# AlerianEmperor/Voxel-Cone-Tracing

Hardware: AMD Instinct MI355X
Metric: Mcones/s (+ ms per GI pass), Sponza-class 256^3 @1080p (higher is better)
Workload: dtype f32; 1 GPU; procedural atrium (Sponza-class, 257488 tris, seed 1234), 256^3 RGBA8 brick chain, 1920x1080, 6 diffuse + 1 specular cone/px, trace of a resident (GPU-rasterised) G-buffer; voxel_dim=256, width=1920, height=1080, cones_per_pixel=7, bounces=1, anisotropic_mips=False, parallelism=single GPU, trace_variant=0, footprint_records=False, comm_reserved_cus=0, raster_form=direct

## Files before the change

include/vct.h:

```cpp
#ifndef VCT_H_
#define VCT_H_

#include <stddef.h>
#include <stdint.h>

#ifdef __cplusplus
extern "C" {
#endif

#define VCT_ABI_VERSION 7

typedef enum vct_status {
    VCT_OK = 0,
    VCT_ERR_INVALID = -1,
    VCT_ERR_DEVICE = -2,
    VCT_ERR_NO_DEVICE = -3,
    VCT_ERR_NOMEM = -4
} vct_status;

enum {
    VCT_GB_POSITION = 0,
    VCT_GB_NORMAL = 3,
    VCT_GB_TANGENT = 6,
    VCT_GB_BITANGENT = 9,
// ... 160 lines not shown
#define VCT_COMM_ID_BYTES 128
int vct_slab_partition(int32_t height, int32_t world, int32_t rank, int32_t* tile_row0, int32_t* tile_row1,
                       int32_t* rows_per_rank);
int vct_comm_get_unique_id(void* id128);
int vct_comm_init(vct_ctx* ctx, const void* id128, int32_t rank, int32_t world);
int vct_comm_destroy(vct_ctx* ctx);
int vct_comm_slab(vct_ctx* ctx, int32_t* tile_row0, int32_t* tile_row1);
int vct_frame_step(vct_ctx* ctx);
int vct_comm_sync(vct_ctx* ctx);
int vct_comm_set_timeout_ms(vct_ctx* ctx, int32_t milliseconds);
int vct_comm_info(vct_ctx* ctx, int32_t out[4]);
int vct_comm_last_gather_ms(vct_ctx* ctx, float* ms);
int vct_last_row_steps(vct_ctx* ctx, uint64_t* rows, int32_t nrows);
int vct_slab_partition_weighted(const uint64_t* row_cost, int32_t tile_rows, int32_t world, int32_t* starts);
int vct_comm_set_slab_rows(vct_ctx* ctx, const int32_t* starts);
int vct_comm_set_interleaved(vct_ctx* ctx, int32_t on);
int vct_selftest_interleaved(vct_ctx* ctx, int32_t world, uint64_t* mismatches);
int vct_comm_frame(vct_ctx* ctx, void** rgba16f_dev, size_t* bytes);
int vct_comm_download_frame(vct_ctx* ctx, void* out_rgba16f_host);

int vct_download_steps(vct_ctx* ctx, uint8_t* steps);
int vct_download_cones(vct_ctx* ctx, float* cones);
int vct_last_step_count(vct_ctx* ctx, uint64_t* steps);
int vct_last_trace_stats(vct_ctx* ctx, uint64_t out[16]);
int vct_get_stage_counts(vct_ctx* ctx, uint64_t out[8]);
int vct_last_trace_ms(vct_ctx* ctx, float* ms);
int vct_set_trace_timing(vct_ctx* ctx, int32_t on);
int vct_selftest_const_divide(vct_ctx* ctx, float d, uint64_t* mismatches);
int vct_selftest_texel_buffer(vct_ctx* ctx, uint64_t* mismatches);
int vct_selftest_area_divide(vct_ctx* ctx, uint64_t seed, uint64_t count, uint64_t* mismatches);
int vct_get_stream(vct_ctx* ctx, void** hip_stream);
int vct_get_frame_device(vct_ctx* ctx, void** rgba16f_dev, size_t* bytes);

#ifdef __cplusplus
}
#endif
#endif
```

voxel-cone-tracing_amd/__init__.py:

```python
import ctypes as C
import os

import numpy as np

try:
    import torch
except ImportError:
    pass

_HERE = os.path.dirname(os.path.abspath(__file__))
LIB_PATH = os.environ.get("VCT_AMD_LIB") or os.path.join(_HERE, "libvct_amd.so")

GB_PLANES = 23
GB_LINEAR, GB_TILED = 0, 1
MEM_HOST, MEM_DEVICE = 0, 1
VOX_CONSERVATIVE_AVG, VOX_REFERENCE = 0, 1
ABI_VERSION = 7
SHOW_DIFFUSE, SHOW_INDIRECT_DIFFUSE, SHOW_SPECULAR, SHOW_INDIRECT_SPECULAR, SHOW_AMBIENT_OCCLUSION = 1, 2, 4, 8, 16
SHOW_ALL = 31
AOV_INDIRECT_DIFFUSE, AOV_INDIRECT_SPECULAR, AOV_DIRECT = 1, 2, 4
VOXVIEW_CURRENT, VOXVIEW_RADIANCE, VOXVIEW_ALBEDO, VOXVIEW_NORMAL = 0, 1, 2, 3
QUERY_SORT_CELLS = 1
POINT_QUERY_MAX = 1 << 26
APERTURE_DIFFUSE, APERTURE_SPECULAR = 0, 1
# ... 556 lines not shown
        v = C.c_int32()
        self._ck(_lib.vct_get_frames_in_flight(self._h, None, None, C.byref(v)), "vct_get_frames_in_flight")
        return bool(v.value)

    def select_frame_slot(self, slot):
        self._ck(_lib.vct_select_frame_slot(self._h, slot), "vct_select_frame_slot")

    def steps(self):
        out = np.zeros((self.cfg.height * self.cfg.width, 7), np.uint8)
        self._ck(_lib.vct_download_steps(self._h, _ptr(out)), "vct_download_steps")
        return out

    def cones(self):
        out = np.zeros((self.cfg.height * self.cfg.width, 7, 4), np.float32)
        self._ck(_lib.vct_download_cones(self._h, _ptr(out)), "vct_download_cones")
        return out

    def last_step_count(self):
        v = C.c_uint64()
        self._ck(_lib.vct_last_step_count(self._h, C.byref(v)), "vct_last_step_count")
        return v.value

    def last_trace_stats(self):
        v = (C.c_uint64 * 16)()
        self._ck(_lib.vct_last_trace_stats(self._h, v), "vct_last_trace_stats")
        keys = ("wave_steps", "lane_steps", "coop_zero", "coop_hit", "fallback", "fallback_lanes", "fallback_fits",
                "greedy_blocks", "greedy_le2", "greedy_le3", "greedy_le4", "quads_live", "quads_fit333", "quads_same",
                "quadrants_live", "quadrants_fit444")
        return dict(zip(keys, (int(x) for x in v)))

    def stage_counts(self):
        v = (C.c_uint64 * 8)()
        self._ck(_lib.vct_get_stage_counts(self._h, v), "vct_get_stage_counts")
        return dict(zip(("triangles", "vox_candidates", "march_division", "accumulator_bricks", "touched_bricks",
                         "comm_reserved_cus", "raster_form", "vox_items"), (int(x) for x in v)))

    def set_trace_timing(self, on=True):
        self._ck(_lib.vct_set_trace_timing(self._h, int(bool(on))), "vct_set_trace_timing")

    def last_trace_ms(self):
        v = C.c_float()
        self._ck(_lib.vct_last_trace_ms(self._h, C.byref(v)), "vct_last_trace_ms")
        return v.value

    def selftest_const_divide(self, d):
        v = C.c_uint64()
        self._ck(_lib.vct_selftest_const_divide(self._h, float(d), C.byref(v)), "vct_selftest_const_divide")
        return v.value

    def selftest_area_divide(self, seed, count):
        v = C.c_uint64()
# ... 17 lines not shown
```

voxel-cone-tracing_amd/csrc/vct_api_trace.hip:

```cpp
#include <algorithm>
#include <map>
#include <mutex>

#include "vct_ctx.h"
#include "vct_divisors.h"

namespace {

int build_steps(const vct_config& cfg, float tan_half, std::vector<VctStep>& out) {
    out.clear();
    const int maxl = vct_ilog2(cfg.voxel_dim);
    const float vs = cfg.grid_world_size / (float)cfg.voxel_dim;
    float dist = vs;
    while (dist < cfg.max_distance) {
        if ((int)out.size() >= VCT_MAX_STEPS) return -1;
        VctStep s;
        const float diameter = fmaxf(vs, 2.0f * tan_half * dist);
        const float lod = log2f(diameter / vs);
        s.dist = dist;
        s.occ_den = 1.0f + 0.03f * diameter;
        s.occ_rcp = 1.0f / s.occ_den;
        float lam = lod;
        if (!(lam > 0.0f)) {
            s.two_levels = 0; s.level = 0; s.level2 = 0; s.frac = 0.0f;
// ... 174 lines not shown
    const uint32_t aov_which = pack_rows ? 0u : c->aov_which;
    const bool half = c->diffuse_rate == 2;
    bool half_march = false;
    if (half) {
        if (row0 != 0 || row1 != vct_tiles_y(c) || row_stride > 1 || pack_rows)
            return vct_fail(c, VCT_ERR_INVALID, "trace: diffuse rate 2 traces whole frames only (no slabs, tile-row ranges or interleaved rows)");
        if (variant != 0 || c->cfg.anisotropic_mips || c->vol.want_cells || c->comm || !cur(c).dr_ind)
            return vct_fail(c, VCT_ERR_INVALID, "trace: diffuse rate 2 needs the default trace kernel on a single-GPU context");
        p.comp = component_word(c->show_mask, aov_which);
        p.aov = aov_which ? cur(c).aov.get() : nullptr;
        half_march = ((p.comp >> VCT_COMP_GROUPS_SHIFT) & 1u) != 0u;
        if (half_march) {
            p.dr_ind = cur(c).dr_ind.get(); p.dr_coarse = cur(c).dr_coarse.get(); p.dr_anchor = cur(c).dr_anchor.get();
            p.dr_list = cur(c).dr_list.get(); p.dr_ctr = cur(c).dr_ctr.get();
            p.dr_waves = c->diffuse_rate_waves;
        }
    } else if (c->show_mask != VCT_SHOW_ALL || aov_which) {
        if (variant != 0)
            return vct_fail(c, VCT_ERR_INVALID, "lighting components / per-component outputs need the default trace kernel (config.trace_variant 0)");
        p.comp = component_word(c->show_mask, aov_which);
        p.aov = aov_which ? cur(c).aov.get() : nullptr;
    }
#if defined(VCT_STATS) && VCT_STATS
    HIP_TRY(c, hipMemsetAsync(c->stats.get(), 0, 16 * sizeof(unsigned long long), cur(c).stream.get()));
#endif
    if (compacting) {
        const size_t nt = (size_t)vct_tiles_x(c) * vct_tiles_y(c);
        HIP_TRY(c, c->vt_pix.reserve(nt * 64 + 4));
        p.vt_pix = c->vt_pix.get();
        p.vt_count = c->vt_pix.get() + nt * 64;
        HIP_TRY(c, hipMemsetAsync(p.vt_count, 0, sizeof(uint32_t), cur(c).stream.get()));
    }
    if (c->time_traces) HIP_TRY(c, hipEventRecord(cur(c).ev0.get(), cur(c).stream.get()));
    const hipEvent_t marks[3] = {cur(c).dr_ev[0].get(), cur(c).dr_ev[1].get(), cur(c).dr_ev[2].get()};
    HIP_TRY(c, vct_launch_trace(p, variant, cur(c).stream.get(), &c->last_march_form,
                                half_march && c->time_traces ? marks : nullptr));
    if (c->time_traces) HIP_TRY(c, hipEventRecord(cur(c).ev1.get(), cur(c).stream.get()));
    cur(c).last_trace_timed = c->time_traces;
    cur(c).last_trace_half = half_march;
    cur(c).last_row0 = row0;
    cur(c).last_row1 = row1;
    cur(c).last_row_stride = rstride;
    cur(c).have_trace = true;
    cur(c).last_was_screen_trace = true;
    cur(c).last_trace_compacted = compacting;
    return VCT_OK;
}
// ... 253 lines not shown
        HIP_TRY(c, hipMemcpy(v, c->step_counter.get(), sizeof(v), hipMemcpyDeviceToHost));
        for (int i = 0; i < VCT_STEP_COUNTERS; ++i) sum += v[i];
    }
    *steps = sum;
    return VCT_OK;
}

int vct_last_row_steps(vct_ctx* c, uint64_t* rows, int32_t nrows) {
    if (!c || !rows) return VCT_ERR_INVALID;
    if (!cur(c).have_trace || !cur(c).last_was_screen_trace)
        return vct_fail(c, VCT_ERR_INVALID, "vct_last_row_steps: the last march was not a screen trace");
    if (nrows != vct_tiles_y(c)) return vct_fail(c, VCT_ERR_INVALID, "vct_last_row_steps: nrows must be the frame's tile rows, ceil(height / 8)");
    if (c->diffuse_rate == 2 || cur(c).last_trace_half)
        return vct_fail(c, VCT_ERR_INVALID, "vct_last_row_steps: diffuse rate 2 keeps no per-row histogram (its marches are not per tile row)");
    if (cur(c).last_trace_compacted)
        return vct_fail(c, VCT_ERR_INVALID, "vct_last_row_steps: the last trace was compacted (config.trace_variant 4): no per-row histogram");
    HIP_TRY(c, hipSetDevice(c->device));
    std::vector<uint64_t> v;
    PIPE_TRY(row_steps(c, v));
    memcpy(rows, v.data(), (size_t)nrows * sizeof(uint64_t));
    return VCT_OK;
}

int vct_last_trace_stats(vct_ctx* c, uint64_t out[16]) {
    if (!c || !out) return VCT_ERR_INVALID;
#if defined(VCT_STATS) && VCT_STATS
    if (!cur(c).have_trace) return vct_fail(c, VCT_ERR_INVALID, "no trace has run");
    HIP_TRY(c, hipStreamSynchronize(cur(c).stream.get()));
    HIP_TRY(c, hipMemcpy(out, c->stats.get(), 16 * sizeof(uint64_t), hipMemcpyDeviceToHost));
    return VCT_OK;
#else
    return vct_fail(c, VCT_ERR_INVALID, "vct_last_trace_stats: this library was built without -DVCT_STATS=1 "
                                    "(tools/build_ab.sh stats \"-DVCT_STATS=1\")");
#endif
}

int vct_last_trace_ms(vct_ctx* c, float* ms) {
    if (!c || !ms) return VCT_ERR_INVALID;
    if (!cur(c).have_trace) return vct_fail(c, VCT_ERR_INVALID, "no trace has run");
    if (!cur(c).last_trace_timed)
        return vct_fail(c, VCT_ERR_INVALID, "vct_last_trace_ms: the last trace was issued with timing off (vct_set_trace_timing)");
    HIP_TRY(c, hipEventSynchronize(cur(c).ev1.get()));
    HIP_TRY(c, hipEventElapsedTime(ms, cur(c).ev0.get(), cur(c).ev1.get()));
    return VCT_OK;
}

int vct_selftest_const_divide(vct_ctx* c, float d, uint64_t* mismatches) {
    if (!c || !mismatches) return VCT_ERR_INVALID;
    if (!divisor_ok(d)) return vct_fail(c, VCT_ERR_INVALID, "divisor outside the set the FMA division is proven for");
    HIP_TRY(c, hipSetDevice(c->device));
    unsigned long long v[2] = {0, 0};
    PIPE_TRY(selftest_words(c, v, [&](unsigned long long* w, hipStream_t st) { return vct_launch_divide_selftest(d, w, st); }));
// ... 171 lines not shown
```

voxel-cone-tracing_amd/csrc/vct_capi.hip:

```cpp
#include <map>
#include <mutex>
#include <utility>

#include "vct_ctx.h"

namespace {

std::string g_create_error;

bool is_pow2(int v) { return v > 0 && (v & (v - 1)) == 0; }

__global__ void k_spin_stamp(long long ticks, unsigned long long* out) {
    const long long t0 = (long long)wall_clock64();
    while ((long long)wall_clock64() - t0 < ticks) __builtin_amdgcn_s_sleep(16);
    out[0] = wall_clock64();
}
__global__ void k_stamp(unsigned long long* out) { out[1] = wall_clock64(); }

int streams_overlap(vct_ctx* c, hipStream_t base, hipStream_t cand, bool* overlap) {
    int khz = 0;
    if (hipDeviceGetAttribute(&khz, hipDeviceAttributeWallClockRate, c->device) != hipSuccess || khz <= 0) khz = 100000;
    HIP_TRY(c, hipMemsetAsync(c->stats.get(), 0, 2 * sizeof(unsigned long long), base));
    HIP_TRY(c, hipStreamSynchronize(base));
    hipLaunchKernelGGL(k_spin_stamp, dim3(1), dim3(1), 0, base, (long long)khz * 3 / 10, c->stats.get());
// ... 51 lines not shown
    HIP_TRY(c, slot_create(c, c->slots[0], stream));
    const char* rp = getenv("VCT_RASTER_PATH");
    c->raster_form.mode = !rp ? 0 : (rp[0] == 'b' ? 2 : (rp[0] == 'd' ? 1 : 0));
    for (VctEvent& ev : c->raster_form.ev) HIP_TRY(c, ev.create());
    if (const char* fr = getenv("VCT_FOOTPRINT_RECORDS")) c->vol.want_cells = fr[0] == '1';
    if (const char* tc = getenv("VCT_BIN_TEST_CAPS")) {
        unsigned a = 0, b = 0;
        if (sscanf(tc, "%u,%u", &a, &b) == 2) { c->raster_form.bin_test_caps[0] = a; c->raster_form.bin_test_caps[1] = b; }
    }
    VctChain& vol = c->vol;
    vol.V = cfg->voxel_dim;
    vol.nlev = vct_ilog2(vol.V) + 1;
    vol.chain_texels = vct_chain_texels(vol.V);
    HIP_TRY(c, vol.chain.alloc(vol.chain_texels));
    HIP_TRY(c, hipMemsetAsync(vol.chain.get(), 0, vol.chain_texels * 4, cur(c).stream.get()));
    const size_t npix = (size_t)cfg->width * cfg->height;
    if (cfg->anisotropic_mips) {
        const size_t n = 6 * (vol.chain_texels - vol.nvox());
        HIP_TRY(c, vol.aniso.alloc(n));
        HIP_TRY(c, hipMemsetAsync(vol.aniso.get(), 0, n * 4, cur(c).stream.get()));
    }
    HIP_TRY(c, c->step_counter.alloc(VCT_STEP_COUNTERS));
    HIP_TRY(c, hipMemsetAsync(c->step_counter.get(), 0, VCT_STEP_COUNTERS * sizeof(unsigned long long), cur(c).stream.get()));
    HIP_TRY(c, c->stats.alloc(16));
    HIP_TRY(c, hipMemsetAsync(c->stats.get(), 0, 16 * sizeof(unsigned long long), cur(c).stream.get()));
    HIP_TRY(c, c->steps_dev.alloc(2 * VCT_MAX_STEPS));
    {
        std::vector<uint32_t> lut(1024);
        for (uint32_t i = 0; i < 1024u; ++i) lut[i] = vct_spread3(i) << 2;
        HIP_TRY(c, c->spread_lut.alloc(lut.size()));
        HIP_TRY(c, hipMemcpy(c->spread_lut.get(), lut.data(), lut.size() * sizeof(uint32_t), hipMemcpyHostToDevice));
    }
    if (cfg->debug_outputs) {
        HIP_TRY(c, c->dbg_steps.alloc(npix * 7));
        HIP_TRY(c, c->dbg_cones.alloc(npix * 28));
        HIP_TRY(c, hipMemsetAsync(c->dbg_steps.get(), 0, npix * 7, cur(c).stream.get()));
        HIP_TRY(c, hipMemsetAsync(c->dbg_cones.get(), 0, npix * 28 * sizeof(float), cur(c).stream.get()));
    }
    HIP_TRY(c, hipStreamSynchronize(cur(c).stream.get()));
    static std::mutex lock;
    static std::map<int, unsigned long long> verdict;
    std::lock_guard<std::mutex> g(lock);
    auto it = verdict.find(c->device);
    if (it == verdict.end()) {
        uint64_t bad = 0;
        PIPE_TRY(vct_selftest_texel_buffer(c, &bad));
        it = verdict.emplace(c->device, bad).first;
    }
// ... 283 lines not shown
```

voxel-cone-tracing_amd/csrc/vct_trace.hip:

```cpp
#include <hip/hip_fp16.h>

#include "../../include/vct.h"
#include "vct_internal.h"
#include "vct_texel.h"


namespace {

struct F3 { float x, y, z; };
struct F4 { float x, y, z, w; };

__device__ __forceinline__ F3 f3(float x, float y, float z) { return {x, y, z}; }
__device__ __forceinline__ float dot3(F3 a, F3 b) { return a.x * b.x + a.y * b.y + a.z * b.z; }
__device__ __forceinline__ F3 cross3(F3 a, F3 b) {
    return {a.y * b.z - a.z * b.y, a.z * b.x - a.x * b.z, a.x * b.y - a.y * b.x};
}
__device__ __forceinline__ float div_rn(float a, float b) { return a / b; }
__device__ __forceinline__ float sqrt_rn(float a) { return __builtin_sqrtf(a); }
__device__ __forceinline__ F3 normalize3(F3 a) {
    const float l = sqrt_rn(dot3(a, a));
    return {div_rn(a.x, l), div_rn(a.y, l), div_rn(a.z, l)};
}
__device__ __forceinline__ F3 reflect3(F3 I, F3 N) {
    const float d = 2.0f * dot3(N, I);
// ... 37 lines not shown
__device__ __forceinline__ float unorm8_of(uint32_t t) {
    if (LOOSE) return (float)((t >> SHIFT) & 0xffu) * 0x1.010102p-8f;
    return vct_unorm8_to_float((t >> SHIFT) & 0xffu);
}

#ifndef VCT_STATS
#define VCT_STATS 0
#endif
struct MarchStats {
    uint32_t wave_steps;
    uint32_t lane_steps;
    uint32_t coop_zero;
    uint32_t coop_hit;
    uint32_t fallback;
    uint32_t fallback_lanes;
    uint32_t fallback_fits;
    uint32_t greedy_blocks, greedy_le2, greedy_le3, greedy_le4;
    uint32_t two_blocks;
    uint32_t quads_live;
    uint32_t quads_fit333;
    uint32_t quads_same;
    uint32_t quadrants_live;
    uint32_t quadrants_fit444;
};

template <bool WRAP, bool COOP, bool LOOSE = false, bool CELLS = false, bool PRIO = false>
__device__ __forceinline__ F4 sample_level(const uint32_t* __restrict__ chain, const VctLevelRef lv,
                                           float ux, float uy, float uz, bool act, unsigned long long am,
                                           float4* __restrict__ blk, const LaneBlock& lb, MarchStats& ms,
                                           const char* __restrict__ cells = nullptr) {
    if (PRIO) __builtin_amdgcn_s_setprio(1);
    const int m = lv.m;
    const float fN = lv.fN;
    const float u = fmaf(ux, fN, -0.5f), v = fmaf(uy, fN, -0.5f), w = fmaf(uz, fN, -0.5f);
    const float fu = floorf(u), fv = floorf(v), fw = floorf(w);
    const float a = u - fu, b = v - fv, c = w - fw;
    const int i0 = (int)fu, j0 = (int)fv, k0 = (int)fw;
    const uint32_t* __restrict__ base = chain + lv.off;
    const uint32_t MX = lv.mask_x, MY = MX << 1, MZ = MX << 2;
    const vct_v4i32 tb = level_texel_buffer(base);

    F4 r = {0.0f, 0.0f, 0.0f, 0.0f};
    bool coop = false;
    int ax = 0, ay = 0, az = 0, dx = 0, dy = 0, dz = 0;
    if (COOP) {
        const int src = ((am >> 27) & 1ull) ? 27 : (int)__ffsll((long long)am) - 1;
        ax = __builtin_amdgcn_readlane(i0, src) - 1;
// ... 7 lines not shown
    if (COOP && coop) {
        uint32_t idx;
        if (WRAP) {
            const uint32_t m4 = (uint32_t)m << 2;
            const uint32_t sax = spread_byte(lb.lut, ax, m4) >> 2;
            const uint32_t say = spread_byte(lb.lut, ay, m4) >> 1;
            const uint32_t saz = spread_byte(lb.lut, az, m4);
            idx = (((sax | ~MX) + lb.sbx) & MX) | (((say | ~MY) + lb.sby) & MY) |
                  (((saz | ~MZ) + lb.sbz) & MZ);
        } else {
            const int x = min(max(ax + (lb.lane & 3), 0), m);
            const int y = min(max(ay + ((lb.lane >> 2) & 3), 0), m);
            const int z = min(max(az + (lb.lane >> 4), 0), m);
            idx = vct_morton3((uint32_t)x, (uint32_t)y, (uint32_t)z);
        }
        const float4 d = texel_f32(tb, idx);
        if (PRIO) __builtin_amdgcn_s_setprio(0);
        const bool any_texel = ballot64((__float_as_uint(d.x) | __float_as_uint(d.y) | __float_as_uint(d.z) | __float_as_uint(d.w)) != 0u) != 0ull;
        if (VCT_STATS) { if (any_texel) ++ms.coop_hit; else ++ms.coop_zero; }
        if (any_texel) {
            blk[lb.lane] = d;
            wave_sync();
            const int slot = act ? (dz * 4 + dy) * 4 + dx : 0;
            const float4* q = blk + slot;
            const float a0 = 1.0f - a, b0 = 1.0f - b, c0 = 1.0f - c;
            const float ab00 = a0 * b0, ab10 = a * b0, ab01 = a0 * b, ab11 = a * b;
            {
                const float4 t0 = q[0], t1 = q[1], t2 = q[4], t3 = q[5];
                const float w0 = ab00 * c0, w1 = ab10 * c0, w2 = ab01 * c0, w3 = ab11 * c0;
#define VCT_ACC(ch) r.ch = w0 * t0.ch; r.ch = fmaf(w1, t1.ch, r.ch); r.ch = fmaf(w2, t2.ch, r.ch); r.ch = fmaf(w3, t3.ch, r.ch);
                VCT_ACC(x) VCT_ACC(y) VCT_ACC(z) VCT_ACC(w)
#undef VCT_ACC
            }
            __builtin_amdgcn_sched_barrier(0);
            {
                const float4 t4 = q[16], t5 = q[17], t6 = q[20], t7 = q[21];
                wave_sync();
                const float w4 = ab00 * c, w5 = ab10 * c, w6 = ab01 * c, w7 = ab11 * c;
#define VCT_ACC(ch) r.ch = fmaf(w4, t4.ch, r.ch); r.ch = fmaf(w5, t5.ch, r.ch); r.ch = fmaf(w6, t6.ch, r.ch); r.ch = fmaf(w7, t7.ch, r.ch);
                VCT_ACC(x) VCT_ACC(y) VCT_ACC(z) VCT_ACC(w)
#undef VCT_ACC
            }
        }
    } else {
      if (VCT_STATS) {
          ++ms.fallback; ms.fallback_lanes += (uint32_t)__popcll(am);
          int lo[3] = {act ? i0 : 0x7fffffff, act ? j0 : 0x7fffffff, act ? k0 : 0x7fffffff};
          int hi[3] = {act ? i0 : -0x7fffffff, act ? j0 : -0x7fffffff, act ? k0 : -0x7fffffff};
          for (int off = 32; off > 0; off >>= 1)
              for (int q = 0; q < 3; ++q) { lo[q] = min(lo[q], __shfl_xor(lo[q], off)); hi[q] = max(hi[q], __shfl_xor(hi[q], off)); }
          if (hi[0] - lo[0] <= 2 && hi[1] - lo[1] <= 2 && hi[2] - lo[2] <= 2) ++ms.fallback_fits;
          unsigned long long pending = am;
          int nb = 0;
          while (pending != 0ull && nb < 16) {
              const int src = (int)__ffsll((long long)pending) - 1;
              const int bx = __builtin_amdgcn_readlane(i0, src) - 1, by = __builtin_amdgcn_readlane(j0, src) - 1,
                        bz = __builtin_amdgcn_readlane(k0, src) - 1;
              const bool in = (uint32_t)(i0 - bx) <= 2u && (uint32_t)(j0 - by) <= 2u && (uint32_t)(k0 - bz) <= 2u;
              pending &= ~ballot64(in);
              ++nb;
          }
          int qlo[3] = {act ? i0 : 0x7fffffff, act ? j0 : 0x7fffffff, act ? k0 : 0x7fffffff};
          int qhi[3] = {act ? i0 : -0x7fffffff, act ? j0 : -0x7fffffff, act ? k0 : -0x7fffffff};
          bool qany = act;
          auto widen = [&](int off) {
// ... 85 lines not shown
                t[6] = base[mx0 | my1 | mz1]; t[7] = base[mx1 | my1 | mz1];
            }
            if (PRIO) __builtin_amdgcn_s_setprio(0);
            const float a0 = 1.0f - a, b0 = 1.0f - b, c0 = 1.0f - c;
            const float wg[8] = {(a0 * b0) * c0, (a * b0) * c0, (a0 * b) * c0, (a * b) * c0,
                                 (a0 * b0) * c,  (a * b0) * c,  (a0 * b) * c,  (a * b) * c};
            r.x = wg[0] * unorm8_of<0, LOOSE>(t[0]);
            r.y = wg[0] * unorm8_of<8, LOOSE>(t[0]);
            r.z = wg[0] * unorm8_of<16, LOOSE>(t[0]);
            r.w = wg[0] * unorm8_of<24, LOOSE>(t[0]);
#pragma unroll
            for (int i = 1; i < 8; ++i) {
                r.x = fmaf(wg[i], unorm8_of<0, LOOSE>(t[i]), r.x);
                r.y = fmaf(wg[i], unorm8_of<8, LOOSE>(t[i]), r.y);
                r.z = fmaf(wg[i], unorm8_of<16, LOOSE>(t[i]), r.z);
                r.w = fmaf(wg[i], unorm8_of<24, LOOSE>(t[i]), r.w);
            }
        }
      }
    }
    return r;
}

struct AnisoCone {
    float wx, wy, wz;
    bool nx, ny, nz;
};

template <bool WRAP, bool COOP>
__device__ __forceinline__ F4 sample_aniso(const VctTraceParams& p, const VctLevelRef lv, float ux,
                                           float uy, float uz, bool act, unsigned long long m,
                                           float4* __restrict__ blk, const LaneBlock& lb, const AnisoCone& ac,
                                           MarchStats& ms) {
    auto chain_of = [&](int d) { return p.aniso + (size_t)d * p.aniso_stride - p.level_off[1]; };
    const unsigned long long mx = ballot64(ac.nx) & m, my = ballot64(ac.ny) & m, mz = ballot64(ac.nz) & m;
    F4 tx, ty, tz;
    bool done = false;
    if (COOP && WRAP) {
        const int mm = lv.m;
        const float fN = lv.fN;
        const float u = fmaf(ux, fN, -0.5f), v = fmaf(uy, fN, -0.5f), w = fmaf(uz, fN, -0.5f);
        const float fu = floorf(u), fv = floorf(v), fw = floorf(w);
        const float a = u - fu, b = v - fv, c = w - fw;
        const int i0 = (int)fu, j0 = (int)fv, k0 = (int)fw;
        const int src = ((m >> 27) & 1ull) ? 27 : (int)__ffsll((long long)m) - 1;
        const int ax = __builtin_amdgcn_readlane(i0, src) - 1;
// ... 75 lines not shown
    r.w = ac.wx * tx.w; r.w = fmaf(ac.wy, ty.w, r.w); r.w = fmaf(ac.wz, tz.w, r.w);
    return r;
}

typedef const __attribute__((address_space(4))) VctStep* StepTable;

__device__ __forceinline__ VctStep load_step(StepTable t, int k) {
    VctStep s;
    s.dist = t[k].dist; s.occ_rcp = t[k].occ_rcp; s.occ_den = t[k].occ_den; s.frac = t[k].frac;
    s.level = t[k].level; s.level2 = t[k].level2; s.two_levels = t[k].two_levels; s.omf = t[k].omf;
    s.l1.off = t[k].l1.off; s.l1.mask_x = t[k].l1.mask_x; s.l1.fN = t[k].l1.fN; s.l1.m = t[k].l1.m;
    s.l2.off = t[k].l2.off; s.l2.mask_x = t[k].l2.mask_x; s.l2.fN = t[k].l2.fN; s.l2.m = t[k].l2.m;
    return s;
}

#define VCT_MARCH_STEP(st, act, live)                                                                        \
        const float px = start.x + dir.x * st.dist; \
        const float py = start.y + dir.y * st.dist; \
        const float pz = start.z + dir.z * st.dist; \
        const float ux = fmaf(div_const<FASTDIV>(px, p.half_G_aux, p.half_G_rcp), 0.5f, 0.5f); \
        const float uy = fmaf(div_const<FASTDIV>(py, p.half_G_aux, p.half_G_rcp), 0.5f, 0.5f); \
        const float uz = fmaf(div_const<FASTDIV>(pz, p.half_G_aux, p.half_G_rcp), 0.5f, 0.5f); \
        F4 vc = (ANISO && st.level >= 1) ? sample_aniso<WRAP, COOP>(p, st.l1, ux, uy, uz, act, live, blk, lb, ac, ms) \
                                         : sample_level<WRAP, COOP, FASTDIV == 2, CELLS, PRIO>(p.chain, st.l1, ux, uy, uz, act, live, blk, lb, ms, p.cells_biased); \
        if (st.two_levels) { \
            const F4 t2 = ANISO ? sample_aniso<WRAP, COOP>(p, st.l2, ux, uy, uz, act, live, blk + 64, lb, ac, ms) \
                                : sample_level<WRAP, COOP, FASTDIV == 2, CELLS, PRIO>(p.chain, st.l2, ux, uy, uz, act, live, blk + 64, lb, ms, p.cells_biased); \
            const float g = st.omf;       \
            vc.x = fmaf(st.frac, t2.x, g * vc.x); \
            vc.y = fmaf(st.frac, t2.y, g * vc.y); \
            vc.z = fmaf(st.frac, t2.z, g * vc.z); \
            vc.w = fmaf(st.frac, t2.w, g * vc.w); \
        } \
        if (act) { \
            const float oma = 1.0f - alpha; \
            cr = fmaf(oma, vc.x, cr); \
            cg = fmaf(oma, vc.y, cg); \
            cb = fmaf(oma, vc.z, cb); \
            occ = occ + div_const<FASTDIV>(oma * vc.w, st.occ_den, st.occ_rcp); \
            alpha = fmaf(oma, vc.w, alpha); \
            ++steps; \
        }

template <bool WRAP, int FASTDIV, bool COOP, bool ANISO = false, bool CELLS = false, bool PRIO = false>
__device__ __forceinline__ F4 cone_march(const VctTraceParams& p, bool alive, F3 start, F3 dir,
                                         const VctStep* tab_global, int n,
                                         float4* __restrict__ blk, const LaneBlock& lb,
                                         int& steps_out, MarchStats& ms) {
    const StepTable tab = (StepTable)tab_global;
    float cr = 0.0f, cg = 0.0f, cb = 0.0f, occ = 0.0f;
    int steps = 0;
    AnisoCone ac = {0.0f, 0.0f, 0.0f, false, false, false};
    if (ANISO) {
        ac.wx = dir.x * dir.x; ac.wy = dir.y * dir.y; ac.wz = dir.z * dir.z;
        ac.nx = !(dir.x >= 0.0f); ac.ny = !(dir.y >= 0.0f); ac.nz = !(dir.z >= 0.0f);
    }
    const float wx = start.x + dir.x * p.vs, wy = start.y + dir.y * p.vs, wz = start.z + dir.z * p.vs;
    float alpha = fmaf(wx, 0.0f, fmaf(wy, 0.0f, fmaf(wz, 0.0f, 0.0f)));
    const unsigned long long alive_mask = ballot64(alive);
    if constexpr (!ANISO) {
    auto march_step = [&](const VctStep& st, const bool act, const unsigned long long live) { VCT_MARCH_STEP(st, act, live) };
    VctStep ea = load_step(tab, 0), eb = ea;
    for (int k = 0; k < n;) {
        {
            const bool act = alive && (alpha < p.max_alpha);
            const unsigned long long live = ballot64(alpha < p.max_alpha) & alive_mask;
            if (live == 0ull) break;
            if (VCT_STATS) { ++ms.wave_steps; ms.lane_steps += (uint32_t)__popcll(live); }
            eb = load_step(tab, k + 1 < n ? k + 1 : k);
            march_step(ea, act, live);
            if (++k >= n) break;
// ... 8 lines not shown
            ++k;
        }
    }
    } else {
    VctStep nxt = load_step(tab, 0);
    for (int k = 0; k < n; ++k) {
        const bool act = alive && (alpha < p.max_alpha);
        const unsigned long long live = ballot64(alpha < p.max_alpha) & alive_mask;
        if (live == 0ull) break;
        if (VCT_STATS) { ++ms.wave_steps; ms.lane_steps += (uint32_t)__popcll(live); }
        const VctStep st = nxt;
        nxt = load_step(tab, k + 1 < n ? k + 1 : k);
        VCT_MARCH_STEP(st, act, live)
    }
    }
    if (alive && steps == 0 && alpha != alpha && n > 0 && 0.0f < p.max_alpha) {
        cr = cg = cb = occ = __builtin_nanf("");
        steps = 1;
    }
    steps_out = steps;
    return {cr, cg, cb, occ};
}

__device__ __forceinline__ void flush_stats(const VctTraceParams& p, const MarchStats& ms, int lane) {
    if (VCT_STATS && p.stats && lane == 0) {
        const uint32_t v[16] = {ms.wave_steps, ms.lane_steps, ms.coop_zero, ms.coop_hit, ms.fallback,
                                ms.fallback_lanes, ms.fallback_fits, ms.greedy_blocks, ms.greedy_le2, ms.greedy_le3,
                                ms.greedy_le4, ms.quads_live, ms.quads_fit333, ms.quads_same, ms.quadrants_live,
                                ms.quadrants_fit444};
        for (int i = 0; i < 16; ++i)
            if (v[i]) atomicAdd(p.stats + i, (unsigned long long)v[i]);
    }
}

__constant__ float kConeDirs[18] = {0.0f, 0.0f, 1.0f,
                                    0.0f, 0.866025f, 0.5f,
                                    0.823639f, 0.267617f, 0.5f,
                                    0.509037f, -0.700629f, 0.5f,
                                    -0.509037f, -0.700629f, 0.5f,
                                    -0.823639f, 0.267617f, 0.5f};
__constant__ float kConeWeights[6] = {0.25f, 0.15f, 0.15f, 0.15f, 0.15f, 0.15f};

__device__ __forceinline__ LaneBlock make_lane_block(const VctTraceParams& p, int lane) {
    LaneBlock lb;
    lb.lane = lane;
    lb.lut = (SpreadLut)p.spread_lut; lb.lut_vec = p.spread_lut;
    lb.sbx = vct_spread3((uint32_t)lane & 3u);
    lb.sby = vct_spread3(((uint32_t)lane >> 2) & 3u) << 1;
// ... 201 lines not shown
    __shared__ int lds_done;
    __shared__ int lds_steps;
    const int lane = threadIdx.x & 63;
    const int wave = __builtin_amdgcn_readfirstlane((int)(threadIdx.x >> 6));
    float4* blk = &lds_blk[wave][0][0];
    if (threadIdx.x == 0) { lds_done = 0; lds_steps = 0; }
    __syncthreads();

    const int ntiles = p.ntiles;
    const int ti = xcd_remap((int)blockIdx.x, (int)gridDim.x);
    if (ti >= ntiles) return;
    constexpr bool compact = COMPACT;
    uint32_t cpix = 0u;
    if (compact) {
        if ((uint32_t)ti >= *p.vt_count) {
            if (threadIdx.x == 0) p.tile_steps[p.tile_row0 * p.tiles_x + ti] = 0u;
            return;
        }
        cpix = p.vt_pix[(size_t)ti * 64 + lane];
    }

    const LaneBlock lb = make_lane_block(p, lane);
    MarchStats ms = {};

    int lrow = 0, tile0 = p.tile_row0 * p.tiles_x + ti;
    if (p.row_stride > 1) {
        lrow = ti / p.tiles_x;
        tile0 = (p.tile_row0 + lrow * p.row_stride) * p.tiles_x + (ti - lrow * p.tiles_x);
    }
    const bool cvalid = !compact || cpix != 0xffffffffu;
    const int tile = compact ? (cvalid ? (int)(cpix >> 6) : 0) : tile0;
    const int ty = tile / p.tiles_x, tx = tile - ty * p.tiles_x;
    const int oy = p.pack_rows ? (p.row_stride > 1 ? lrow : ty - p.tile_row0) : ty;
    const int plane_ = compact ? (int)(cpix & 63u) : lane;
    auto fresh_lane = [&]() { int l = plane_; asm volatile("" : "+v"(l)); return l; };
    auto pixel_index = [&]() {
        const int l = fresh_lane();
        return (size_t)(oy * VCT_TILE + (l >> 3)) * p.width + (tx * VCT_TILE + (l & 7));
    };
    auto gbuf_ptr = [&](int l) {
        return p.gbuf + (size_t)tile * (VCT_GB_NPLANES * VCT_TILE_PIX) + l;
    };
    const int x = tx * VCT_TILE + (plane_ & 7), y = ty * VCT_TILE + (plane_ >> 3);
    const float* gb = gbuf_ptr(plane_);
    const bool in_frame = cvalid && (x < p.width) && (y < p.height);
    const bool alive = in_frame && !(gb_plane(gb, 18) < 0.5f);
    int total = 0;
    const uint32_t groups = COMP ? (uint32_t)__builtin_amdgcn_readfirstlane((int)p.comp) >> VCT_COMP_GROUPS_SHIFT : 3u;
    const int n_diffuse = (groups & 1u) ? p.n_diffuse : 0, n_specular = (groups & 2u) ? p.n_specular : 0;
    if (HALF && wave < VCT_SPLIT - 1) {
    } else if (wave < VCT_SPLIT - 1) {
        F3 start, k0, k1, k2;
        cone_frame_from_gbuffer(gb, p.vs, start, k0, k1, k2);
#pragma unroll 1
        for (int i = wave * VCT_CONES_PER_WAVE; i < wave * VCT_CONES_PER_WAVE + VCT_CONES_PER_WAVE; ++i) {
            int st;
            const F4 c = cone_march<WRAP, FASTDIV, true, ANISO, CELLS, PRIO>(p, alive, start, cone_dir(k0, k1, k2, i),
                                                                p.steps_diffuse, n_diffuse, blk, lb, st, ms);
            total += st;
            lds_cone[i][lane] = make_float4(c.x, c.y, c.z, c.w);
            store_debug_cone(p, pixel_index, i, c, st, alive, in_frame);
        }
    } else {
        if (!PRIO && p.spec_prio) __builtin_amdgcn_s_setprio(1);
        const F3 P = gb_planes3(gb, 0), Nw = gb_planes3(gb, 3), N = gb_planes3(gb, 12);
        const F3 start = cone_start(P, Nw, p.vs);
        int st6;
        const F4 sc = cone_march<WRAP, FASTDIV, true, ANISO, CELLS, PRIO>(p, alive, start, specular_dir(P, N, p.cam),
                                                             p.steps_specular, n_specular, blk, lb, st6, ms);
        total += st6;
        lds_cone[6][lane] = make_float4(sc.x, sc.y, sc.z, sc.w);
        store_debug_cone(p, pixel_index, 6, sc, st6, alive, in_frame);
    }
    for (int off = 32; off > 0; off >>= 1) total += __shfl_xor(total, off);
    if (lane == 0) atomicAdd(&lds_steps, total);
    flush_stats(p, ms, lane);

    __threadfence_block();
    int arrived = 0;
    if (lane == 0) arrived = atomicAdd(&lds_done, 1);
    arrived = __builtin_amdgcn_readfirstlane(arrived);
    if (arrived != VCT_SPLIT - 1) return;
    __threadfence_block();
    if (lane == 0) p.tile_steps[tile0] = (uint32_t)lds_steps;

    const float* gb3 = gbuf_ptr(fresh_lane());
    if (in_frame) {
        F4 ind = {0.0f, 0.0f, 0.0f, 0.0f};
        if (HALF) {
            const float4 v = p.dr_ind[pixel_index()];
            ind = {v.x, v.y, v.z, v.w};
        } else {
#pragma unroll
            for (int i = 0; i < 6; ++i) ind = fold_cone(ind, i, lds_cone[i][lane]);
        }
        composite<COMP>(p, gb3, ind, lds_cone[6][lane], alive, pixel_index);
    }
}

// ... 674 lines not shown
```

Before: 26900 Mcones/s.

## Reuse cooperatively loaded 4x4x4 brick across steps in second-level sampling

```diff
diff --git a/include/vct.h b/include/vct.h
--- a/include/vct.h
+++ b/include/vct.h
@@ -206,7 +206,7 @@
 int vct_download_steps(vct_ctx* ctx, uint8_t* steps);
 int vct_download_cones(vct_ctx* ctx, float* cones);
 int vct_last_step_count(vct_ctx* ctx, uint64_t* steps);
-int vct_last_trace_stats(vct_ctx* ctx, uint64_t out[16]);
+int vct_last_trace_stats(vct_ctx* ctx, uint64_t out[32]);
 int vct_get_stage_counts(vct_ctx* ctx, uint64_t out[8]);
 int vct_last_trace_ms(vct_ctx* ctx, float* ms);
 int vct_set_trace_timing(vct_ctx* ctx, int32_t on);
diff --git a/voxel-cone-tracing_amd/__init__.py b/voxel-cone-tracing_amd/__init__.py
--- a/voxel-cone-tracing_amd/__init__.py
+++ b/voxel-cone-tracing_amd/__init__.py
@@ -602,11 +602,13 @@
         return v.value
 
     def last_trace_stats(self):
-        v = (C.c_uint64 * 16)()
+        v = (C.c_uint64 * 32)()
         self._ck(_lib.vct_last_trace_stats(self._h, v), "vct_last_trace_stats")
         keys = ("wave_steps", "lane_steps", "coop_zero", "coop_hit", "fallback", "fallback_lanes", "fallback_fits",
                 "greedy_blocks", "greedy_le2", "greedy_le3", "greedy_le4", "quads_live", "quads_fit333", "quads_same",
                 "quadrants_live", "quadrants_fit444")
+        keys += tuple(f"reuse_{c}_{wave}_{level}" for wave in ("diffuse", "specular") for level in ("first", "second")
+                      for c in ("candidates", "hits", "hits_zero", "equal_anchor"))
         return dict(zip(keys, (int(x) for x in v)))
 
     def stage_counts(self):
diff --git a/voxel-cone-tracing_amd/csrc/vct_api_trace.hip b/voxel-cone-tracing_amd/csrc/vct_api_trace.hip
--- a/voxel-cone-tracing_amd/csrc/vct_api_trace.hip
+++ b/voxel-cone-tracing_amd/csrc/vct_api_trace.hip
@@ -220,7 +220,7 @@
         p.aov = aov_which ? cur(c).aov.get() : nullptr;
     }
 #if defined(VCT_STATS) && VCT_STATS
-    HIP_TRY(c, hipMemsetAsync(c->stats.get(), 0, 16 * sizeof(unsigned long long), cur(c).stream.get()));
+    HIP_TRY(c, hipMemsetAsync(c->stats.get(), 0, 32 * sizeof(unsigned long long), cur(c).stream.get()));
 #endif
     if (compacting) {
         const size_t nt = (size_t)vct_tiles_x(c) * vct_tiles_y(c);
@@ -520,12 +520,12 @@
     return VCT_OK;
 }
 
-int vct_last_trace_stats(vct_ctx* c, uint64_t out[16]) {
+int vct_last_trace_stats(vct_ctx* c, uint64_t out[32]) {
     if (!c || !out) return VCT_ERR_INVALID;
 #if defined(VCT_STATS) && VCT_STATS
     if (!cur(c).have_trace) return vct_fail(c, VCT_ERR_INVALID, "no trace has run");
     HIP_TRY(c, hipStreamSynchronize(cur(c).stream.get()));
-    HIP_TRY(c, hipMemcpy(out, c->stats.get(), 16 * sizeof(uint64_t), hipMemcpyDeviceToHost));
+    HIP_TRY(c, hipMemcpy(out, c->stats.get(), 32 * sizeof(uint64_t), hipMemcpyDeviceToHost));
     return VCT_OK;
 #else
     return vct_fail(c, VCT_ERR_INVALID, "vct_last_trace_stats: this library was built without -DVCT_STATS=1 "
diff --git a/voxel-cone-tracing_amd/csrc/vct_capi.hip b/voxel-cone-tracing_amd/csrc/vct_capi.hip
--- a/voxel-cone-tracing_amd/csrc/vct_capi.hip
+++ b/voxel-cone-tracing_amd/csrc/vct_capi.hip
@@ -97,8 +97,8 @@
     }
     HIP_TRY(c, c->step_counter.alloc(VCT_STEP_COUNTERS));
     HIP_TRY(c, hipMemsetAsync(c->step_counter.get(), 0, VCT_STEP_COUNTERS * sizeof(unsigned long long), cur(c).stream.get()));
-    HIP_TRY(c, c->stats.alloc(16));
-    HIP_TRY(c, hipMemsetAsync(c->stats.get(), 0, 16 * sizeof(unsigned long long), cur(c).stream.get()));
+    HIP_TRY(c, c->stats.alloc(32));
+    HIP_TRY(c, hipMemsetAsync(c->stats.get(), 0, 32 * sizeof(unsigned long long), cur(c).stream.get()));
     HIP_TRY(c, c->steps_dev.alloc(2 * VCT_MAX_STEPS));
     {
         std::vector<uint32_t> lut(1024);
diff --git a/voxel-cone-tracing_amd/csrc/vct_trace.hip b/voxel-cone-tracing_amd/csrc/vct_trace.hip
--- a/voxel-cone-tracing_amd/csrc/vct_trace.hip
+++ b/voxel-cone-tracing_amd/csrc/vct_trace.hip
@@ -83,7 +83,41 @@
     uint32_t quads_same;
     uint32_t quadrants_live;
     uint32_t quadrants_fit444;
+    uint32_t reuse[2][4];
 };
+
+#ifndef VCT_REUSE
+#define VCT_REUSE 1
+#endif
+#define VCT_NO_BLOCK 0xfffffff0u
+struct BlockDesc {
+    uint32_t id;
+    int ax, ay, az;
+};
+__device__ __forceinline__ BlockDesc no_block() { return {VCT_NO_BLOCK, 0, 0, 0}; }
+
+__device__ __forceinline__ F4 gather_block(const float4* q, float a, float b, float c) {
+    F4 r;
+    const float a0 = 1.0f - a, b0 = 1.0f - b, c0 = 1.0f - c;
+    const float ab00 = a0 * b0, ab10 = a * b0, ab01 = a0 * b, ab11 = a * b;
+    {
+        const float4 t0 = q[0], t1 = q[1], t2 = q[4], t3 = q[5];
+        const float w0 = ab00 * c0, w1 = ab10 * c0, w2 = ab01 * c0, w3 = ab11 * c0;
+#define VCT_ACC(ch) r.ch = w0 * t0.ch; r.ch = fmaf(w1, t1.ch, r.ch); r.ch = fmaf(w2, t2.ch, r.ch); r.ch = fmaf(w3, t3.ch, r.ch);
+        VCT_ACC(x) VCT_ACC(y) VCT_ACC(z) VCT_ACC(w)
+#undef VCT_ACC
+    }
+    __builtin_amdgcn_sched_barrier(0);
+    {
+        const float4 t4 = q[16], t5 = q[17], t6 = q[20], t7 = q[21];
+        wave_sync();
+        const float w4 = ab00 * c, w5 = ab10 * c, w6 = ab01 * c, w7 = ab11 * c;
+#define VCT_ACC(ch) r.ch = fmaf(w4, t4.ch, r.ch); r.ch = fmaf(w5, t5.ch, r.ch); r.ch = fmaf(w6, t6.ch, r.ch); r.ch = fmaf(w7, t7.ch, r.ch);
+        VCT_ACC(x) VCT_ACC(y) VCT_ACC(z) VCT_ACC(w)
+#undef VCT_ACC
+    }
+    return r;
+}
 
 template <bool WRAP, bool COOP, bool LOOSE = false, bool CELLS = false, bool PRIO = false>
 __device__ __forceinline__ F4 sample_level(const uint32_t* __restrict__ chain, const VctLevelRef lv,
@@ -137,25 +171,7 @@
             blk[lb.lane] = d;
             wave_sync();
             const int slot = act ? (dz * 4 + dy) * 4 + dx : 0;
-            const float4* q = blk + slot;
-            const float a0 = 1.0f - a, b0 = 1.0f - b, c0 = 1.0f - c;
-            const float ab00 = a0 * b0, ab10 = a * b0, ab01 = a0 * b, ab11 = a * b;
-            {
-                const float4 t0 = q[0], t1 = q[1], t2 = q[4], t3 = q[5];
-                const float w0 = ab00 * c0, w1 = ab10 * c0, w2 = ab01 * c0, w3 = ab11 * c0;
-#define VCT_ACC(ch) r.ch = w0 * t0.ch; r.ch = fmaf(w1, t1.ch, r.ch); r.ch = fmaf(w2, t2.ch, r.ch); r.ch = fmaf(w3, t3.ch, r.ch);
-                VCT_ACC(x) VCT_ACC(y) VCT_ACC(z) VCT_ACC(w)
-#undef VCT_ACC
-            }
-            __builtin_amdgcn_sched_barrier(0);
-            {
-                const float4 t4 = q[16], t5 = q[17], t6 = q[20], t7 = q[21];
-                wave_sync();
-                const float w4 = ab00 * c, w5 = ab10 * c, w6 = ab01 * c, w7 = ab11 * c;
-#define VCT_ACC(ch) r.ch = fmaf(w4, t4.ch, r.ch); r.ch = fmaf(w5, t5.ch, r.ch); r.ch = fmaf(w6, t6.ch, r.ch); r.ch = fmaf(w7, t7.ch, r.ch);
-                VCT_ACC(x) VCT_ACC(y) VCT_ACC(z) VCT_ACC(w)
-#undef VCT_ACC
-            }
+            r = gather_block(blk + slot, a, b, c);
         }
     } else {
       if (VCT_STATS) {
@@ -287,6 +303,83 @@
     return r;
 }
 
+template <bool WRAP, bool LOOSE, bool PRIO, int SLAB>
+__device__ __forceinline__ F4 sample_level_reuse(const uint32_t* __restrict__ chain, const VctLevelRef lv,
+                                                 float ux, float uy, float uz, bool act, unsigned long long am,
+                                                 float4* __restrict__ blk, const LaneBlock& lb, MarchStats& ms,
+                                                 BlockDesc& held) {
+    if (PRIO) __builtin_amdgcn_s_setprio(1);
+    const int m = lv.m;
+    const float fN = lv.fN;
+    const float u = fmaf(ux, fN, -0.5f), v = fmaf(uy, fN, -0.5f), w = fmaf(uz, fN, -0.5f);
+    const float fu = floorf(u), fv = floorf(v), fw = floorf(w);
+    const float a = u - fu, b = v - fv, c = w - fw;
+    const int i0 = (int)fu, j0 = (int)fv, k0 = (int)fw;
+    int mode = 0, at = 0;
+    if ((held.id & ~1u) == lv.off) {
+        const BlockDesc cd = held;
+        const int dx = i0 - cd.ax, dy = j0 - cd.ay, dz = k0 - cd.az;
+        const uint32_t far = max(max((uint32_t)dx, (uint32_t)dy), (uint32_t)dz);
+        const unsigned long long out = ballot64(far > 2u) & am;
+        if (VCT_STATS) {
+            const int src = ((am >> 27) & 1ull) ? 27 : (int)__ffsll((long long)am) - 1;
+            ++ms.reuse[SLAB][0];
+            if (out == 0ull) { ++ms.reuse[SLAB][1]; if (!(cd.id & 1u)) ++ms.reuse[SLAB][2]; }
+            if (__builtin_amdgcn_readlane(i0, src) - 1 == cd.ax && __builtin_amdgcn_readlane(j0, src) - 1 == cd.ay &&
+                __builtin_amdgcn_readlane(k0, src) - 1 == cd.az) ++ms.reuse[SLAB][3];
+        }
+        if (out == 0ull) {
+            if (PRIO) __builtin_amdgcn_s_setprio(0);
+            mode = 1 + (int)(cd.id & 1u);
+            at = (act ? (dz * 4 + dy) * 4 + dx : 0) + 64;
+        }
+    }
+    if (mode == 0) {
+        const int src = ((am >> 27) & 1ull) ? 27 : (int)__ffsll((long long)am) - 1;
+        const int ax = __builtin_amdgcn_readlane(i0, src) - 1;
+        const int ay = __builtin_amdgcn_readlane(j0, src) - 1;
+        const int az = __builtin_amdgcn_readlane(k0, src) - 1;
+        const int dx = i0 - ax, dy = j0 - ay, dz = k0 - az;
+        const uint32_t far = max(max((uint32_t)dx, (uint32_t)dy), (uint32_t)dz);
+        const unsigned long long out = ballot64(far > 2u) & am;
+        if (out == 0ull) {
+            const uint32_t MX = lv.mask_x, MY = MX << 1, MZ = MX << 2;
+            const uint32_t m4 = (uint32_t)m << 2;
+            const uint32_t sax = spread_byte(lb.lut, ax, m4) >> 2;
+            const uint32_t say = spread_byte(lb.lut, ay, m4) >> 1;
+            const uint32_t saz = spread_byte(lb.lut, az, m4);
+            const uint32_t idx = (((sax | ~MX) + lb.sbx) & MX) | (((say | ~MY) + lb.sby) & MY) |
+                                 (((saz | ~MZ) + lb.sbz) & MZ);
+            const float4 d = texel_f32(level_texel_buffer(chain + lv.off), idx);
+            if (PRIO) __builtin_amdgcn_s_setprio(0);
+            const unsigned long long any_texel = ballot64((__float_as_uint(d.x) | __float_as_uint(d.y) | __float_as_uint(d.z) | __float_as_uint(d.w)) != 0u);
+            if (VCT_STATS) { if (any_texel != 0ull) ++ms.coop_hit; else ++ms.coop_zero; }
+            mode = any_texel != 0ull ? 2 : 1;
+            if (SLAB == 1) held = {lv.off | (uint32_t)(mode - 1), ax, ay, az};
+            if (mode == 2) {
+                blk[SLAB * 64 + lb.lane] = d;
+                wave_sync();
+                at = (act ? (dz * 4 + dy) * 4 + dx : 0) + SLAB * 64;
+            }
+        }
+    }
+    if (mode == 2) return gather_block(blk + at, a, b, c);
+    if (mode == 1) return {0.0f, 0.0f, 0.0f, 0.0f};
+    return sample_level<WRAP, false, LOOSE, false, PRIO>(chain, lv, ux, uy, uz, act, am, blk, lb, ms);
+}
+
+template <bool WRAP, bool COOP, bool LOOSE, bool CELLS, bool PRIO, bool REUSE, int SLAB>
+__device__ __forceinline__ F4 sample_step_level(const VctTraceParams& p, const VctLevelRef lv, float ux, float uy, float uz,
+                                                bool act, unsigned long long am, float4* __restrict__ blk,
+                                                const LaneBlock& lb, MarchStats& ms, BlockDesc& held) {
+    if constexpr (REUSE) {
+        static_assert(WRAP && COOP && !CELLS, "block reuse: cooperative sampler, GL_REPEAT, no footprint records");
+        return sample_level_reuse<WRAP, LOOSE, PRIO, SLAB>(p.chain, lv, ux, uy, uz, act, am, blk, lb, ms, held);
+    } else {
+        return sample_level<WRAP, COOP, LOOSE, CELLS, PRIO>(p.chain, lv, ux, uy, uz, act, am, blk + SLAB * 64, lb, ms, p.cells_biased);
+    }
+}
+
 struct AnisoCone {
     float wx, wy, wz;
     bool nx, ny, nz;
@@ -408,10 +501,10 @@
         const float uy = fmaf(div_const<FASTDIV>(py, p.half_G_aux, p.half_G_rcp), 0.5f, 0.5f); \
         const float uz = fmaf(div_const<FASTDIV>(pz, p.half_G_aux, p.half_G_rcp), 0.5f, 0.5f); \
         F4 vc = (ANISO && st.level >= 1) ? sample_aniso<WRAP, COOP>(p, st.l1, ux, uy, uz, act, live, blk, lb, ac, ms) \
-                                         : sample_level<WRAP, COOP, FASTDIV == 2, CELLS, PRIO>(p.chain, st.l1, ux, uy, uz, act, live, blk, lb, ms, p.cells_biased); \
+                                         : sample_step_level<WRAP, COOP, FASTDIV == 2, CELLS, PRIO, REUSE, 0>(p, st.l1, ux, uy, uz, act, live, blk, lb, ms, held); \
         if (st.two_levels) { \
             const F4 t2 = ANISO ? sample_aniso<WRAP, COOP>(p, st.l2, ux, uy, uz, act, live, blk + 64, lb, ac, ms) \
-                                : sample_level<WRAP, COOP, FASTDIV == 2, CELLS, PRIO>(p.chain, st.l2, ux, uy, uz, act, live, blk + 64, lb, ms, p.cells_biased); \
+                                : sample_step_level<WRAP, COOP, FASTDIV == 2, CELLS, PRIO, REUSE, 1>(p, st.l2, ux, uy, uz, act, live, blk, lb, ms, held); \
             const float g = st.omf;       \
             vc.x = fmaf(st.frac, t2.x, g * vc.x); \
             vc.y = fmaf(st.frac, t2.y, g * vc.y); \
@@ -428,11 +521,11 @@
             ++steps; \
         }
 
-template <bool WRAP, int FASTDIV, bool COOP, bool ANISO = false, bool CELLS = false, bool PRIO = false>
+template <bool WRAP, int FASTDIV, bool COOP, bool ANISO, bool CELLS, bool PRIO, bool REUSE>
 __device__ __forceinline__ F4 cone_march(const VctTraceParams& p, bool alive, F3 start, F3 dir,
                                          const VctStep* tab_global, int n,
                                          float4* __restrict__ blk, const LaneBlock& lb,
-                                         int& steps_out, MarchStats& ms) {
+                                         int& steps_out, MarchStats& ms, BlockDesc& held) {
     const StepTable tab = (StepTable)tab_global;
     float cr = 0.0f, cg = 0.0f, cb = 0.0f, occ = 0.0f;
     int steps = 0;
@@ -487,8 +580,19 @@
     return {cr, cg, cb, occ};
 }
 
-__device__ __forceinline__ void flush_stats(const VctTraceParams& p, const MarchStats& ms, int lane) {
+template <bool WRAP, int FASTDIV, bool COOP, bool ANISO = false, bool CELLS = false, bool PRIO = false>
+__device__ __forceinline__ F4 cone_march(const VctTraceParams& p, bool alive, F3 start, F3 dir,
+                                         const VctStep* tab_global, int n,
+                                         float4* __restrict__ blk, const LaneBlock& lb,
+                                         int& steps_out, MarchStats& ms) {
+    BlockDesc none = no_block();
+    return cone_march<WRAP, FASTDIV, COOP, ANISO, CELLS, PRIO, false>(p, alive, start, dir, tab_global, n, blk, lb, steps_out, ms, none);
+}
+
+__device__ __forceinline__ void flush_stats(const VctTraceParams& p, const MarchStats& ms, int lane, bool specular = false) {
     if (VCT_STATS && p.stats && lane == 0) {
+        for (int i = 0; i < 8; ++i)
+            if (ms.reuse[i >> 2][i & 3]) atomicAdd(p.stats + 16 + (specular ? 8 : 0) + i, (unsigned long long)ms.reuse[i >> 2][i & 3]);
         const uint32_t v[16] = {ms.wave_steps, ms.lane_steps, ms.coop_zero, ms.coop_hit, ms.fallback,
                                 ms.fallback_lanes, ms.fallback_fits, ms.greedy_blocks, ms.greedy_le2, ms.greedy_le3,
                                 ms.greedy_le4, ms.quads_live, ms.quads_fit333, ms.quads_same, ms.quadrants_live,
@@ -736,6 +840,8 @@
 
     const LaneBlock lb = make_lane_block(p, lane);
     MarchStats ms = {};
+    constexpr bool REUSE = VCT_REUSE && WRAP && !ANISO && !CELLS && !COMPACT;
+    BlockDesc held = no_block();
 
     int lrow = 0, tile0 = p.tile_row0 * p.tiles_x + ti;
     if (p.row_stride > 1) {
@@ -769,8 +875,8 @@
 #pragma unroll 1
         for (int i = wave * VCT_CONES_PER_WAVE; i < wave * VCT_CONES_PER_WAVE + VCT_CONES_PER_WAVE; ++i) {
             int st;
-            const F4 c = cone_march<WRAP, FASTDIV, true, ANISO, CELLS, PRIO>(p, alive, start, cone_dir(k0, k1, k2, i),
-                                                                p.steps_diffuse, n_diffuse, blk, lb, st, ms);
+            const F4 c = cone_march<WRAP, FASTDIV, true, ANISO, CELLS, PRIO, REUSE>(p, alive, start, cone_dir(k0, k1, k2, i),
+                                                                       p.steps_diffuse, n_diffuse, blk, lb, st, ms, held);
             total += st;
             lds_cone[i][lane] = make_float4(c.x, c.y, c.z, c.w);
             store_debug_cone(p, pixel_index, i, c, st, alive, in_frame);
@@ -780,15 +886,15 @@
         const F3 P = gb_planes3(gb, 0), Nw = gb_planes3(gb, 3), N = gb_planes3(gb, 12);
         const F3 start = cone_start(P, Nw, p.vs);
         int st6;
-        const F4 sc = cone_march<WRAP, FASTDIV, true, ANISO, CELLS, PRIO>(p, alive, start, specular_dir(P, N, p.cam),
-                                                             p.steps_specular, n_specular, blk, lb, st6, ms);
+        const F4 sc = cone_march<WRAP, FASTDIV, true, ANISO, CELLS, PRIO, REUSE>(p, alive, start, specular_dir(P, N, p.cam),
+                                                                    p.steps_specular, n_specular, blk, lb, st6, ms, held);
         total += st6;
         lds_cone[6][lane] = make_float4(sc.x, sc.y, sc.z, sc.w);
         store_debug_cone(p, pixel_index, 6, sc, st6, alive, in_frame);
     }
     for (int off = 32; off > 0; off >>= 1) total += __shfl_xor(total, off);
     if (lane == 0) atomicAdd(&lds_steps, total);
-    flush_stats(p, ms, lane);
+    flush_stats(p, ms, lane, wave == VCT_SPLIT - 1);
 
     __threadfence_block();
     int arrived = 0;
```

Result: faster. 27240 Mcones/s (median of 6 runs) (+1.3%).
